# david8862/tf-keras-deeplabv3p-model-set

Hardware: AMD Instinct MI355X
Metric: images/sec (513x513, 21-class) MobileNetV2-DeepLabV3+ OS=16 training step (higher is better)
Workload: dtype f32

## Files before the change

tf-keras-deeplabv3p-model-set_amd/csrc/pw_gemm.h:

```cpp
#pragma once
#include "common.h"

struct GemmParams {
  const float* A; int lda;
  const float* scale; const float* shift; int act;
  const float* B; int ldb;
  const float* bias;
  float* Y; int ldy;
  float* partials;
  int M, K, N;
  int accumulate;
  int num_m_tiles;
  int ksplit, kchunk;
  int stagger;
  int b_kn;
  const float* bb_z; int bb_ldz;
  const float* bb_scale; const float* bb_shift; const float* bb_mean; const float* bb_invstd; int bb_act;
  int g_RH, g_RW, g_SH, g_SW, g_C, g_kw, g_mul, g_ay, g_ax, g_d, g_shift;
  uint32_t g_cmagic;
  int g_kwmagic;
  const unsigned short* Bsp; int bsp_pitch; long long bsp_plane;
  const float* f_z; int f_ldz; const float* f_scale; const float* f_shift; const float* f_mean; const float* f_invstd;
  const float* f_coef; int f_act; float* f_dz; int f_lddz;
};
```

tf-keras-deeplabv3p-model-set_amd/csrc/pw_split.hip:

```cpp
#include "common.h"
#include "pw_gemm.h"
#include "sb_common.h"

__global__ __launch_bounds__(256) void split_bf16x3_kernel(const float* src, unsigned short* dst, const long long* table) {
  const long long* e = table + (size_t)blockIdx.x * 6;
  const long long soff = e[0], doff = e[4];
  const int rows = (int)e[1], cols = (int)e[2], ld = (int)e[3], pitch = (int)e[5];
  const int p8 = pitch / 8;
  const long long plane = (long long)rows * pitch;
  for (long long i = (long long)blockIdx.y * 256 + threadIdx.x; i < (long long)rows * p8; i += (long long)gridDim.y * 256) {
    const int r = (int)(i / p8), c = (int)(i - (long long)r * p8) * 8;
    const long long so = soff + (long long)r * ld + c;
    float v[8];
    if (c + 8 <= cols && (so & 3) == 0) {
      const float4 a = *reinterpret_cast<const float4*>(src + so), b = *reinterpret_cast<const float4*>(src + so + 4);
      v[0] = a.x; v[1] = a.y; v[2] = a.z; v[3] = a.w; v[4] = b.x; v[5] = b.y; v[6] = b.z; v[7] = b.w;
    } else {
#pragma unroll
      for (int k = 0; k < 8; ++k) v[k] = c + k < cols ? src[so + k] : 0.f;
    }
    uint4 h, m, l;
    split2(v[0], v[1], h.x, m.x, l.x);
    split2(v[2], v[3], h.y, m.y, l.y);
    split2(v[4], v[5], h.z, m.z, l.z);
// ... 712 lines not shown
    default: if (mi == 1) launch_sbp_one<8, STATS, 1, BNB>(p, grid, st); else launch_sbp_one<8, STATS, 2, BNB>(p, grid, st); break;
  }
#undef DL3P_SBP
}

void dl3p_launch_gemm_sbp(const GemmParams& p, bool stats, bool bnb, int nt, int mi, dim3 grid, hipStream_t st) {
  if (bnb) launch_sbp_nt<true, true>(p, nt, mi, grid, st);
  else if (stats) launch_sbp_nt<true, false>(p, nt, mi, grid, st);
  else launch_sbp_nt<false, false>(p, nt, mi, grid, st);
}

template <int NT, bool STATS, int MI, bool BNB, bool GA, int WM>
static void launch_sb_one(const GemmParams& p, dim3 grid, hipStream_t st) {
  constexpr int BM = 64 * MI * WM, BN = 16 * NT;
  constexpr int OPER = 3 * (BM + BN) * SB_PB * 2;
  constexpr int TPP = NT < 4 ? NT : 4;
  constexpr int ES = 4 * WM * 16 * MI * (16 * TPP + 4) * 4;
  constexpr int RED = STATS ? 2 * 4 * WM * BN * 4 : 0;
  constexpr size_t lds = (size_t)(OPER > ES ? OPER : ES) + RED;
  static bool attr_set = false;
  if (!attr_set) {
    if (lds > 64 * 1024)
      (void)hipFuncSetAttribute((const void*)pw_gemm_sb_kernel<NT, STATS, MI, BNB, GA, WM>, hipFuncAttributeMaxDynamicSharedMemorySize, (int)lds);
    attr_set = true;
  }
  dl3p_launch(pw_gemm_sb_kernel<NT, STATS, MI, BNB, GA, WM>, grid, dim3(256 * WM), lds, st, p);
}

template <bool STATS, int MI, bool BNB, bool GA>
static void launch_sb_mi(const GemmParams& p, int nt, dim3 grid, hipStream_t st) {
  switch (nt) {
    case 1: launch_sb_one<1, STATS, MI, BNB, GA, 1>(p, grid, st); break;
    case 2: launch_sb_one<2, STATS, MI, BNB, GA, 1>(p, grid, st); break;
    case 3: launch_sb_one<3, STATS, MI, BNB, GA, 1>(p, grid, st); break;
    case 4: launch_sb_one<4, STATS, MI, BNB, GA, 1>(p, grid, st); break;
    case 5: launch_sb_one<5, STATS, MI, BNB, GA, 1>(p, grid, st); break;
    case 6: launch_sb_one<6, STATS, MI, BNB, GA, 1>(p, grid, st); break;
    case 7: launch_sb_one<7, STATS, MI, BNB, GA, 1>(p, grid, st); break;
    default: launch_sb_one<8, STATS, MI, BNB, GA, 1>(p, grid, st); break;
  }
}

template <bool STATS, bool BNB>
static void launch_sb_wide(const GemmParams& p, int nt, int mi, int wm, dim3 grid, hipStream_t st) {
#define DL3P_SBW(N_, M_, W_) if (nt == N_ && mi == M_ && wm == W_) { launch_sb_one<N_, STATS, M_, BNB, false, W_>(p, grid, st); return; }
  DL3P_SBW(16, 2, 1) DL3P_SBW(16, 1, 2) DL3P_SBW(16, 2, 2) DL3P_SBW(12, 2, 1) DL3P_SBW(12, 2, 2) DL3P_SBW(8, 2, 2) DL3P_SBW(16, 1, 1)
#undef DL3P_SBW
  launch_sb_one<16, STATS, 2, BNB, false, 1>(p, grid, st);
}

bool dl3p_sb_wide_config(int nt, int mi, int wm) {
  static const int ok[][3] = {{16, 2, 1}, {16, 1, 2}, {16, 2, 2}, {12, 2, 1}, {12, 2, 2}, {8, 2, 2}, {16, 1, 1}};
  for (auto& c : ok) if (c[0] == nt && c[1] == mi && c[2] == wm) return true;
  return false;
}

void dl3p_launch_gemm_sb(const GemmParams& p, bool stats, bool bnb, bool ga, int nt, int mi, int wm, dim3 grid, hipStream_t st) {
  if (wm > 1 || nt > 8) {
    if (bnb) launch_sb_wide<true, true>(p, nt, mi, wm, grid, st);
    else if (stats) launch_sb_wide<true, false>(p, nt, mi, wm, grid, st);
    else launch_sb_wide<false, false>(p, nt, mi, wm, grid, st);
    return;
  }
#define DL3P_SB(S, B, G) \
  { if (mi == 1) launch_sb_mi<S, 1, B, G>(p, nt, grid, st); else launch_sb_mi<S, 2, B, G>(p, nt, grid, st); return; }
  if (ga) {
    if (stats) DL3P_SB(true, false, true) else DL3P_SB(false, false, true)
  }
  if (bnb) DL3P_SB(true, true, false)
  if (stats) DL3P_SB(true, false, false)
  DL3P_SB(false, false, false)
#undef DL3P_SB
}

struct WgradSB {
  const float* X; int ldx; const float* scale; const float* shift; int act;
  const float* DY; int lddy;
  float* slabs;
  int M, K, N;
  int ktiles, ntiles, mrows;
  int k_base;
  int g_RH, g_RW, g_SH, g_SW, g_C, g_kw, g_mul, g_ay, g_ax, g_d;
  float g_invRW, g_invRH;
};

__device__ __forceinline__ int sb_divmod(int a, int d, float inv, int* r) {
  int q = (int)((float)a * inv);
  int rem = a - q * d;
  if (rem < 0) { --q; rem += d; }
  if (rem >= d) { ++q; rem -= d; }
  *r = rem;
  return q;
}

typedef short s16x4w __attribute__((ext_vector_type(4)));
__device__ __forceinline__ s16x4w tr_read16(const unsigned short* lds_ptr) {
  return __builtin_amdgcn_ds_read_tr16_b64_v4i16((s16x4w __attribute__((address_space(3)))*)lds_ptr);
}

template <int KF, int NW, int WN, bool GX = false>
__global__ __launch_bounds__(256, 2) void pw_wgrad_sb_kernel(WgradSB p) {
  constexpr int TK = 64 * KF, TN = 16 * NW, MS = 32;
  constexpr int KFW = KF * WN, NWW = NW / WN;
  constexpr int XP = TK + 8, DP = TN + 8;
  constexpr int X_PLANE = MS * XP, D_PLANE = MS * DP;
  constexpr int XCPR = TK / 8, DCPR = TN / 8;
  constexpr int XROWS = 256 / XCPR, DROWS = 256 / DCPR;
  constexpr int NXP = MS / XROWS, NDP = MS / DROWS;
  extern __shared__ __attribute__((aligned(16))) unsigned short wg_lds[];
  unsigned short* Xs = wg_lds;
  unsigned short* Ds = wg_lds + 3 * X_PLANE;
  const int t = threadIdx.x, l = t & 63, w = t >> 6;
  const int wk = w / WN, wn = w - wk * WN;
  const int tile = blockIdx.x, kt = tile / p.ntiles, nt = tile - kt * p.ntiles;
  const int k0 = p.k_base + kt * TK, n0 = nt * TN;
  const int mbeg = blockIdx.y * p.mrows, mend = min(p.M, mbeg + p.mrows);
  const int xm = t / XCPR, xc = (t - xm * XCPR) * 8;
  const int dm = t / DCPR, dc = (t - dm * DCPR) * 8;
  const int xk = k0 + xc, dn = n0 + dc;
  const bool xok0 = xk < p.K, xok1 = xk + 4 < p.K, dok0 = dn < p.N, dok1 = dn + 4 < p.N;
  const int xk0 = min(xk, p.K - 4), xk1 = min(xk + 4, p.K - 4), dn0 = min(dn, p.N - 4), dn1 = min(dn + 4, p.N - 4);
  const float* scp = p.scale ? p.scale : p.X;
  const float* shp = p.scale ? p.shift : p.X;
  int gc[2] = {xk0, xk1}, gdy[2] = {0, 0}, gdx[2] = {0, 0};
  if (GX) {
#pragma unroll
    for (int h = 0; h < 2; ++h) {
      const int k = h ? xk1 : xk0;
      const int tap = k / p.g_C, ky = tap / p.g_kw;
      gc[h] = k - tap * p.g_C;
      gdy[h] = p.g_ay + ky * p.g_d;
      gdx[h] = p.g_ax + (tap - ky * p.g_kw) * p.g_d;
    }
  }
  const float4 sc0 = ld4(scp + gc[0]), sc1 = ld4(scp + gc[1]), sh0 = ld4(shp + gc[0]), sh1 = ld4(shp + gc[1]);
  const float act_lo = p.act == DL3P_ACT_NONE ? -DL3P_INF : 0.f;
  const float act_hi = (p.act == DL3P_ACT_NONE || p.act == DL3P_ACT_RELU) ? DL3P_INF : 6.f;
  auto prologue4 = [&](float4 v, float4 sc4, float4 sh4) __attribute__((always_inline)) {
    if (p.scale) v = fma4(v, sc4, sh4);
    if (p.act >= DL3P_ACT_HSWISH) return act_apply4(v, p.act);
    return make_float4(__builtin_amdgcn_fmed3f(v.x, act_lo, act_hi), __builtin_amdgcn_fmed3f(v.y, act_lo, act_hi),
                       __builtin_amdgcn_fmed3f(v.z, act_lo, act_hi), __builtin_amdgcn_fmed3f(v.w, act_lo, act_hi));
  };
  const bool has_pro = p.scale != nullptr || p.act != DL3P_ACT_NONE;
  uint32_t gx_ok = 0;

  f32x4 acc[KFW][NWW];
#pragma unroll
  for (int kf = 0; kf < KFW; ++kf)
#pragma unroll
    for (int ni = 0; ni < NWW; ++ni) acc[kf][ni] = (f32x4){0.f, 0.f, 0.f, 0.f};
  float4 rx[NXP][2], rd[NDP][2];
  auto prefetch = [&](int m0) __attribute__((always_inline)) {
#pragma unroll
    for (int i = 0; i < NXP; ++i) {
      if (GX) {
        const int m = m0 + xm + XROWS * i;
        int x, y;
        const int row = sb_divmod(min(m, p.M - 1), p.g_RW, p.g_invRW, &x);
        const int n = sb_divmod(row, p.g_RH, p.g_invRH, &y);
        const uint32_t img = (uint32_t)n * (uint32_t)(p.g_SH * p.g_SW);
#pragma unroll
        for (int h = 0; h < 2; ++h) {
          const int sy = y * p.g_mul + gdy[h], sx = x * p.g_mul + gdx[h];
          const bool ok = m < mend && sy >= 0 && sx >= 0 && sy < p.g_SH && sx < p.g_SW;
          const uint32_t off = ok ? (img + (uint32_t)(sy * p.g_SW + sx)) * (uint32_t)p.ldx + (uint32_t)gc[h] : 0u;
          rx[i][h] = ld4(p.X + off);
          gx_ok = (gx_ok & ~(1u << (2 * i + h))) | (ok ? (1u << (2 * i + h)) : 0u);
        }
      } else {
        const float* xr = p.X + (size_t)min(m0 + xm + XROWS * i, p.M - 1) * p.ldx;
        rx[i][0] = ld4(xr + xk0); rx[i][1] = ld4(xr + xk1);
      }
    }
#pragma unroll
    for (int i = 0; i < NDP; ++i) {
      const float* dr = p.DY + (size_t)min(m0 + dm + DROWS * i, p.M - 1) * p.lddy;
      rd[i][0] = ld4(dr + dn0); rd[i][1] = ld4(dr + dn1);
    }
  };
  const int g = l >> 4, q = (l & 15) >> 2, pp = l & 3;
  const int r0 = (8 * g + q), r1 = (8 * g + 4 + q);
  const int nsteps = (mend - mbeg + MS - 1) / MS;
  if (nsteps > 0) prefetch(mbeg);
  for (int s = 0; s < nsteps; ++s) {
    const int m0 = mbeg + s * MS;
#pragma unroll
    for (int i = 0; i < NXP; ++i) {
      float4 v0 = rx[i][0], v1 = rx[i][1];
      if (has_pro) { v0 = prologue4(v0, sc0, sh0); v1 = prologue4(v1, sc1, sh1); }
      const bool rok = m0 + xm + XROWS * i < mend;
      const bool ok0 = GX ? ((gx_ok >> (2 * i)) & 1u) != 0 : rok, ok1 = GX ? ((gx_ok >> (2 * i + 1)) & 1u) != 0 : rok;
      if (!(ok0 && xok0)) v0 = zero4();
      if (!(ok1 && xok1)) v1 = zero4();
      uint4 hh, mm, ll;
      split2(v0.x, v0.y, hh.x, mm.x, ll.x);
      split2(v0.z, v0.w, hh.y, mm.y, ll.y);
      split2(v1.x, v1.y, hh.z, mm.z, ll.z);
      split2(v1.z, v1.w, hh.w, mm.w, ll.w);
      unsigned short* d = Xs + (xm + XROWS * i) * XP + xc;
      *reinterpret_cast<uint4*>(d) = hh;
      *reinterpret_cast<uint4*>(d + X_PLANE) = mm;
      *reinterpret_cast<uint4*>(d + 2 * X_PLANE) = ll;
    }
#pragma unroll
    for (int i = 0; i < NDP; ++i) {
      float4 v0 = rd[i][0], v1 = rd[i][1];
      const bool rok = m0 + dm + DROWS * i < mend;
      if (!(rok && dok0)) v0 = zero4();
      if (!(rok && dok1)) v1 = zero4();
      uint4 hh, mm, ll;
      split2(v0.x, v0.y, hh.x, mm.x, ll.x);
      split2(v0.z, v0.w, hh.y, mm.y, ll.y);
      split2(v1.x, v1.y, hh.z, mm.z, ll.z);
      split2(v1.z, v1.w, hh.w, mm.w, ll.w);
      unsigned short* d = Ds + (dm + DROWS * i) * DP + dc;
      *reinterpret_cast<uint4*>(d) = hh;
      *reinterpret_cast<uint4*>(d + D_PLANE) = mm;
      *reinterpret_cast<uint4*>(d + 2 * D_PLANE) = ll;
    }
    lds_barrier();
    prefetch(mbeg + min(s + 1, nsteps - 1) * MS);
    s16x8 af[KFW][3];
#pragma unroll
    for (int kf = 0; kf < KFW; ++kf)
#pragma unroll
      for (int pl = 0; pl < 3; ++pl) {
        const unsigned short* b = Xs + pl * X_PLANE + (wk * KFW + kf) * 16 + 4 * pp;
        const s16x4w a0 = tr_read16(b + r0 * XP), a1 = tr_read16(b + r1 * XP);
        af[kf][pl] = (s16x8){a0[0], a0[1], a0[2], a0[3], a1[0], a1[1], a1[2], a1[3]};
      }
#pragma unroll
    for (int ni = 0; ni < NWW; ++ni) {
      s16x8 bf[3];
#pragma unroll
      for (int pl = 0; pl < 3; ++pl) {
        const unsigned short* b = Ds + pl * D_PLANE + (wn * NWW + ni) * 16 + 4 * pp;
        const s16x4w b0 = tr_read16(b + r0 * DP), b1 = tr_read16(b + r1 * DP);
        bf[pl] = (s16x8){b0[0], b0[1], b0[2], b0[3], b1[0], b1[1], b1[2], b1[3]};
      }
#pragma unroll
      for (int kf = 0; kf < KFW; ++kf) {
        acc[kf][ni] = split_mac(acc[kf][ni], af[kf][0], af[kf][1], af[kf][2], bf[0], bf[1], bf[2]);
      }
    }
    lds_barrier();
  }
  float* slab = p.slabs + (size_t)blockIdx.y * p.K * p.N;
#pragma unroll
  for (int kf = 0; kf < KFW; ++kf)
#pragma unroll
    for (int ni = 0; ni < NWW; ++ni) {
      const int n = n0 + (wn * NWW + ni) * 16 + (l & 15);
#pragma unroll
      for (int j = 0; j < 4; ++j) {
        const int k = k0 + (wk * KFW + kf) * 16 + 4 * g + j;
        if (k < p.K && n < p.N) slab[(size_t)k * p.N + n] = acc[kf][ni][j];
      }
    }
}

int dl3p_wgrad_sb_plan(int M, int K, int N, int max_slabs, int tile, int per_cu, int* kf, int* nw, int* ktiles, int* ntiles, int* mrows) {
  if (M < 1024 || K < 32 || N < 32 || K % 4 || N % 4 || max_slabs < 1) return 0;
  static const int cand[5][2] = {{2, 8}, {1, 8}, {2, 4}, {1, 4}, {2, 16}};
  float best = 1e30f;
  for (int i = 0; i < (tile == 4 ? 5 : 4); ++i) {
    const int tk = 64 * cand[i][0], tn = 16 * cand[i][1];
    const float area = (float)((K + tk - 1) / tk * tk) * (float)((N + tn - 1) / tn * tn);
    const float cost = area * (1.f + 0.5f * (64.f / tk + 64.f / tn));
    if ((tile < 0 && cost < best) || tile == i) { best = cost; *kf = cand[i][0]; *nw = cand[i][1]; }
  }
  *ktiles = (K + 64 * *kf - 1) / (64 * *kf);
  *ntiles = (N + 16 * *nw - 1) / (16 * *nw);
  const int tiles = *ktiles * *ntiles;
  if (per_cu <= 0) per_cu = (*kf == 2 && *nw == 8) ? 2 : 4;
  int s = (DL3P_NUM_CUS * per_cu) / tiles;
  if (s < 1) s = 1;
  const int max_s = (M + 255) / 256;
  if (s > max_s) s = max_s;
  if (s > max_slabs) s = max_slabs;
  const int chunk = ((M + s - 1) / s + 31) / 32 * 32;
  *mrows = chunk;
  return (M + chunk - 1) / chunk;
}

template <int KF, int NW, int WN, bool GX>
static void launch_wgrad_tile(const WgradSB& p, dim3 grid, hipStream_t st) {
  constexpr size_t lds = (size_t)3 * 32 * ((64 * KF + 8) + (16 * NW + 8)) * sizeof(unsigned short);
  static bool attr_set = false;
  if (!attr_set) {
    if (lds > 64 * 1024)
      (void)hipFuncSetAttribute((const void*)pw_wgrad_sb_kernel<KF, NW, WN, GX>, hipFuncAttributeMaxDynamicSharedMemorySize, (int)lds);
    attr_set = true;
  }
  dl3p_launch(pw_wgrad_sb_kernel<KF, NW, WN, GX>, grid, dim3(256), lds, st, p);
}

void dl3p_launch_wgrad_sb(const float* x, int ldx, const float* scale, const float* shift, int act, const float* dy, int lddy,
                          float* slabs, int M, int K, int N, int kf, int nw, int ktiles, int ntiles, int mrows, int splits, hipStream_t st) {
  WgradSB p = {x, ldx, scale, shift, act, dy, lddy, slabs, M, K, N, ktiles, ntiles, mrows, 0};
  const dim3 block(256);
  if (kf == 2 && nw == 8) {
    const int rem = K % 128;
    static const int mixed = getenv("DL3P_WGRAD_SB_MIXED") ? atoi(getenv("DL3P_WGRAD_SB_MIXED")) : 0;
    if (mixed && rem > 0 && rem <= 64 && ktiles > 1) {
      p.ktiles = ktiles - 1;
      launch_wgrad_tile<2, 8, 2, false>(p, dim3(p.ktiles * ntiles, splits), st);
      p.k_base = 128 * (ktiles - 1);
      p.ktiles = 1;
      launch_wgrad_tile<1, 8, 1, false>(p, dim3(ntiles, splits), st);
      return;
    }
    launch_wgrad_tile<2, 8, 2, false>(p, dim3(ktiles * ntiles, splits), st);
  } else if (kf == 2 && nw == 16) launch_wgrad_tile<2, 16, 2, false>(p, dim3(ktiles * ntiles, splits), st);
  else if (kf == 1 && nw == 8) launch_wgrad_tile<1, 8, 1, false>(p, dim3(ktiles * ntiles, splits), st);
  else if (kf == 2 && nw == 4) launch_wgrad_tile<2, 4, 1, false>(p, dim3(ktiles * ntiles, splits), st);
  else launch_wgrad_tile<1, 4, 1, false>(p, dim3(ktiles * ntiles, splits), st);
}

void dl3p_launch_wgrad_sb_gx(const float* x, int ldx, const float* scale, const float* shift, int act, const float* dy, int lddy,
                             float* slabs, int M, int K, int N, const int* geo, int kf, int nw, int ktiles, int ntiles, int mrows, int splits,
                             hipStream_t st) {
  WgradSB p = {x, ldx, scale, shift, act, dy, lddy, slabs, M, K, N, ktiles, ntiles, mrows, 0};
  p.g_RH = geo[0]; p.g_RW = geo[1]; p.g_SH = geo[2]; p.g_SW = geo[3]; p.g_C = geo[4]; p.g_kw = geo[5]; p.g_mul = geo[6];
  p.g_ay = geo[7]; p.g_ax = geo[8]; p.g_d = geo[9];
  p.g_invRW = 1.f / (float)p.g_RW; p.g_invRH = 1.f / (float)p.g_RH;
  const dim3 grid(ktiles * ntiles, splits);
  if (kf == 2 && nw == 8) launch_wgrad_tile<2, 8, 2, true>(p, grid, st);
  else if (kf == 1 && nw == 8) launch_wgrad_tile<1, 8, 1, true>(p, grid, st);
  else if (kf == 2 && nw == 4) launch_wgrad_tile<2, 4, 1, true>(p, grid, st);
  else launch_wgrad_tile<1, 4, 1, true>(p, grid, st);
}
```

tf-keras-deeplabv3p-model-set_amd/csrc/pwconv.hip:

```cpp
#include "common.h"
#include <limits.h>
#include <type_traits>
#include <string.h>

typedef float f32x4 __attribute__((ext_vector_type(4)));

#define BK 32
#define APITCH 36

#include "pw_gemm.h"

#ifndef DL3P_GEMM_PIN_B
#define DL3P_GEMM_PIN_B 1
#endif
template <int NT, bool B_KN, bool STATS, int MI, int BKT, bool BNB = false, bool GA = false>
__global__ __launch_bounds__(256, 2) void pw_gemm_kernel(GemmParams p_in) {
  GemmParams p = p_in;
  int block_y = blockIdx.y;
#ifndef DL3P_NO_SPLITK
  if constexpr (!B_KN && !STATS && !BNB && !GA) {
    if (p.ksplit > 1) {
      const int nbn = (int)gridDim.y / p.ksplit;
      const int z = block_y / nbn;
      block_y -= z * nbn;
// ... 1704 lines not shown
  static const int off = getenv("DL3P_WGRAD_SMALL") ? atoi(getenv("DL3P_WGRAD_SMALL")) == 0 : 0;
  if (off) return false;
  const int kt = ceil_div(K, 16), ntn = ceil_div(N, 16);
  int best = -1, best_tiles = 1 << 30;
  for (int i = 0; i < (int)(sizeof(list) / sizeof(list[0])); ++i)
    if (list[i].kt >= kt && list[i].ntn >= ntn && list[i].kt * list[i].ntn < best_tiles) { best = i; best_tiles = list[i].kt * list[i].ntn; }
  if (best < 0 || best_tiles > 2 * kt * ntn) return false;
  *out = list[best];
  return true;
}

template <bool BNA = false>
static void launch_wgrad_small_any(const WgradParams& p, SmallShape sh, int grid, hipStream_t st) {
#define DL3P_WS(a, b) if (sh.kt == a && sh.ntn == b) { launch_wgrad_small<a, b, BNA>(p, grid, st); return; }
  DL3P_WS(1, 2) DL3P_WS(2, 1) DL3P_WS(2, 2) DL3P_WS(1, 6) DL3P_WS(2, 3) DL3P_WS(2, 4) DL3P_WS(4, 2) DL3P_WS(6, 2)
  DL3P_WS(2, 6) DL3P_WS(2, 9) DL3P_WS(9, 2) DL3P_WS(2, 12) DL3P_WS(12, 2) DL3P_WS(4, 4)
#undef DL3P_WS
}

static void wgrad_pick_tile(int M, int K, int N, int* kw, int* nw) {
  static const int cand[4][2] = {{1, 4}, {2, 4}, {1, 8}, {2, 8}};
  static const int env_force = getenv("DL3P_WGRAD_TILE") ? atoi(getenv("DL3P_WGRAD_TILE")) : -1;
  int force = env_force;
  if (const GemmTuned* e = gemm_tuned_lookup(4, M, K, N)) force = e->nt;
  if (g_wgrad_force_tile >= 0) force = g_wgrad_force_tile;
  if (force < 0 && M < 65536) { *kw = 1; *nw = 4; return; }
  float best = 1e30f;
  for (int i = 0; i < 4; ++i) {
    if (force >= 0 && i != force) continue;
    const int tk = 64 * cand[i][0], tn = 16 * cand[i][1];
    const float area = (float)(ceil_div(K, tk) * tk) * (float)(ceil_div(N, tn) * tn);
    const float cost = area * (1.f + 0.5f * (64.f / tk + 64.f / tn));
    if (cost < best) { best = cost; *kw = cand[i][0]; *nw = cand[i][1]; }
  }
}

static void wgrad_split(int M, int K, int N, int* ktiles, int* ntiles, int* splits, int* mchunk) {
  int kw, nw;
  wgrad_pick_tile(M, K, N, &kw, &nw);
  *ktiles = ceil_div(K, 64 * kw);
  *ntiles = ceil_div(N, 16 * nw);
  const int tiles = *ktiles * *ntiles;
  static const int env_per_cu = getenv("DL3P_WGRAD_PER_CU") ? atoi(getenv("DL3P_WGRAD_PER_CU")) : 4;
  int per_cu = env_per_cu;
  if (const GemmTuned* e = gemm_tuned_lookup(4, M, K, N)) per_cu = e->mi;
  if (g_wgrad_force_per_cu) per_cu = g_wgrad_force_per_cu;
  int s = (DL3P_NUM_CUS * per_cu) / tiles;
  if (s < 1) s = 1;
  int max_s = ceil_div(M, 256);
  if (s > max_s) s = max_s;
  if (s > DL3P_MAX_STAT_ROWS) s = DL3P_MAX_STAT_ROWS;
  int chunk = ceil_div(ceil_div(M, s), 32) * 32;
  *splits = ceil_div(M, chunk);
  *mchunk = chunk;
}

template <bool GX = false, bool BNA = false>
static void launch_wgrad_tiled(const WgradParams& p, int splits, hipStream_t st) {
  int kw, nw;
  wgrad_pick_tile(p.M, p.K, p.N, &kw, &nw);
  const dim3 grid(p.ktiles * p.ntiles, splits), block(256);
  if (kw == 1 && nw == 4) dl3p_launch(pw_wgrad_kernel<1, 4, GX, BNA>, grid, block, 0, st, p);
  else if (kw == 2 && nw == 4) dl3p_launch(pw_wgrad_kernel<2, 4, GX, BNA>, grid, block, 0, st, p);
  else if (kw == 1 && nw == 8) dl3p_launch(pw_wgrad_kernel<1, 8, GX, BNA>, grid, block, 0, st, p);
  else dl3p_launch(pw_wgrad_kernel<2, 8, GX, BNA>, grid, block, 0, st, p);
}

__global__ __launch_bounds__(256) void colsum_kernel(const float* dy, int lddy, long long M, int C, int c4s, int px,
                                                     int nbx, float* partials) {
  const int b = blockIdx.x;
  const int slab = b / nbx;
  const int bx = b - slab * nbx;
  const int pl = threadIdx.x / c4s;
  const int cl = threadIdx.x - pl * c4s;
  const bool active = pl < px;
  const int cbase4 = slab * c4s;
  const int c = (cbase4 + cl) * 4;
  float4 acc[1] = {zero4()};
  if (active)
    for (long long m = (long long)bx * px + pl; m < M; m += (long long)nbx * px) acc[0] = add4(acc[0], ld4(dy + (size_t)m * lddy + c));
  block_reduce_store<1>(acc, active, pl, cl, c4s, px, cbase4, C, partials + (size_t)bx * C);
}

extern "C" size_t dl3p_pwconv_bwd_weight_workspace(int M, int K, int N) {
  if (M <= 0 || K <= 0 || N <= 0) return 0;
  int kt, nt, s, mc;
  wgrad_split(M, K, N, &kt, &nt, &s, &mc);
  size_t a = (size_t)s * K * N;
  SmallShape sh;
  if (wgrad_small_pick(K, N, &sh)) a = (size_t)wgrad_small_grid(M, sh.kt, sh.ntn) * K * N;
  else {
    int kf, nw, kt2, nt2, mrows;
    const size_t s2 = (size_t)wgrad_sb_route(M, K, N, DL3P_MAX_STAT_ROWS, &kf, &nw, &kt2, &nt2, &mrows) * K * N;
    if (s2 > a) a = s2;
  }
  size_t b = (size_t)512 * N;
  return (a > b ? a : b) * sizeof(float);
}

static int pwconv_bwd_weight_impl(const float* x, int ldx, const float* in_scale, const float* in_shift,
                                  int in_act, const float* dy, int lddy, float* gw, float* gb, float* workspace,
                                  size_t workspace_bytes, int M, int K, int N, int* rows_out, void* stream) {
  int rc = check_mat("dl3p_pwconv_bwd_weight", x, ldx, K);
  if (rc) return rc;
  rc = check_mat("dl3p_pwconv_bwd_weight", dy, lddy, N);
  if (rc) return rc;
  DL3P_CHECK_ARG((gw || rows_out) && workspace && aligned16(workspace) && M > 0, "dl3p_pwconv_bwd_weight: bad arguments");
  DL3P_CHECK_ARG(!rows_out || (!gb && !dl3p_pw_tiny_applies(M)),
                 "dl3p_pwconv_bwd_weight_slabs: no bias gradient and more than %d rows (use dl3p_pwconv_bwd_weight)", 64);
  const size_t need = dl3p_pwconv_bwd_weight_workspace(M, K, N);
  if (workspace_bytes < need) {
    dl3p_set_error("dl3p_pwconv_bwd_weight: workspace %zu < %zu bytes", workspace_bytes, need);
    return DL3P_EWORKSPACE;
  }
  hipStream_t st = (hipStream_t)stream;
  if (dl3p_pw_tiny_applies(M)) {
    DL3P_CHECK_ARG(aligned16(gw) && (!gb || aligned16(gb)), "dl3p_pwconv_bwd_weight: gw/gb must be 16-byte aligned");
    dl3p_pw_tiny_wgrad(x, ldx, in_scale, in_shift, in_act, dy, lddy, gw, gb, M, K, N, st);
    DL3P_CHECK_LAUNCH("dl3p_pwconv_bwd_weight");
    return DL3P_OK;
  }
  WgradParams p = {};
  p.X = x; p.ldx = ldx; p.scale = in_scale; p.shift = in_shift; p.act = in_act;
  p.DY = dy; p.lddy = lddy; p.slabs = workspace; p.M = M; p.K = K; p.N = N;
  int splits;
  SmallShape sh;
  if (M >= 16 && wgrad_small_pick(K, N, &sh) && (unsigned long long)M * (unsigned long long)(ldx > lddy ? ldx : lddy) * 4ull < (1ull << 32)) {
    splits = wgrad_small_grid(M, sh.kt, sh.ntn);
    launch_wgrad_small_any(p, sh, splits, st);
  } else {
    int kf, nw, kt2, nt2, mrows, s2 = 0;
    s2 = wgrad_sb_route(M, K, N, workspace_bytes / ((size_t)K * N * 4), &kf, &nw, &kt2, &nt2, &mrows);
    if (s2 > 0) {
      splits = s2;
      dl3p_launch_wgrad_sb(x, ldx, in_scale, in_shift, in_act, dy, lddy, workspace, M, K, N, kf, nw, kt2, nt2, mrows, s2, st);
    } else {
      wgrad_split(M, K, N, &p.ktiles, &p.ntiles, &splits, &p.mchunk);
      launch_wgrad_tiled<false>(p, splits, st);
    }
  }
  DL3P_CHECK_LAUNCH("dl3p_pwconv_bwd_weight");
  if (rows_out) { *rows_out = splits; return DL3P_OK; }
  rc = dl3p_reduce_rows_impl(workspace, splits, (size_t)K * N, gw, 0, st);
  if (rc) return rc;
  if (gb) {
    int c4s, px, nslab;
    pick_lanes(N, &c4s, &px, &nslab);
    long long need_b = ceil_div_ll(M, px);
    int nbx = (int)(need_b < 512 ? need_b : 512);
    hipLaunchKernelGGL(colsum_kernel, dim3(nbx * nslab), dim3(256), 0, st, dy, lddy, (long long)M, N, c4s, px, nbx,
                       workspace);
    DL3P_CHECK_LAUNCH("dl3p_pwconv_bwd_weight(colsum)");
    rc = dl3p_reduce_rows_impl(workspace, nbx, (size_t)N, gb, 0, st);
  }
  return rc;
}

extern "C" int dl3p_pwconv_bwd_weight(const float* x, int ldx, const float* in_scale, const float* in_shift,
                                      int in_act, const float* dy, int lddy, float* gw, float* gb, float* workspace,
                                      size_t workspace_bytes, int M, int K, int N, void* stream) {
  return pwconv_bwd_weight_impl(x, ldx, in_scale, in_shift, in_act, dy, lddy, gw, gb, workspace, workspace_bytes, M, K, N,
                                nullptr, stream);
}

extern "C" int dl3p_pwconv_bwd_weight_slabs(const float* x, int ldx, const float* in_scale, const float* in_shift,
                                            int in_act, const float* dy, int lddy, float* workspace, size_t workspace_bytes,
                                            int* rows_out, int M, int K, int N, void* stream) {
  DL3P_CHECK_ARG(rows_out != nullptr, "dl3p_pwconv_bwd_weight_slabs: rows_out is required");
  return pwconv_bwd_weight_impl(x, ldx, in_scale, in_shift, in_act, dy, lddy, nullptr, nullptr, workspace, workspace_bytes, M, K,
                                N, rows_out, stream);
}


static int wgrad_bn_route(int M, int K, int N) {
  SmallShape sh;
  if (M <= 64 || dl3p_pw_tiny_applies(M) || N % 4 || K % 4) return 0;
  if (M >= 16 && wgrad_small_pick(K, N, &sh)) return (sh.kt == 2 && sh.ntn == 12) ? 0 : 1;
  int kw, nw;
  wgrad_pick_tile(M, K, N, &kw, &nw);
  return (K <= 64 * kw && !(kw == 2 && nw == 8)) ? 2 : 0;
}

extern "C" int dl3p_pwconv_bwd_weight_bn_supported(int M, int K, int N) { return wgrad_bn_route(M, K, N) != 0; }

extern "C" int dl3p_pwconv_bwd_weight_slabs_bn(const float* x, int ldx, const float* in_scale, const float* in_shift,
                                               int in_act, const float* g, int ldg, const float* z, int ldz,
                                               const float* bn_scale, const float* bn_shift, int bn_act,
                                               const float* save_mean, const float* save_invstd, const float* coef,
                                               float* dz, int lddz, float* workspace, size_t workspace_bytes,
                                               int* rows_out, int M, int K, int N, void* stream) {
  const char* fn = "dl3p_pwconv_bwd_weight_slabs_bn";
  int rc = check_mat(fn, x, ldx, K);
  if (rc) return rc;
  rc = check_mat(fn, g, ldg, N);
  if (rc) return rc;
  rc = check_mat(fn, z, ldz, N);
  if (rc) return rc;
  if (dz) {
    rc = check_mat(fn, dz, lddz, N);
    if (rc) return rc;
  }
  DL3P_CHECK_ARG(rows_out && workspace && aligned16(workspace) && save_mean && save_invstd && coef && dz != g,
                 "%s: bad arguments", fn);
  DL3P_CHECK_ARG(dl3p_pwconv_bwd_weight_bn_supported(M, K, N), "%s: shape M=%d K=%d N=%d is not served by the tiled kernel", fn,
                 M, K, N);
  const int ldmax = ldx > ldg ? (ldx > ldz ? ldx : ldz) : (ldg > ldz ? ldg : ldz);
  DL3P_CHECK_ARG((unsigned long long)M * (unsigned long long)(ldmax > lddz ? ldmax : lddz) * 4ull < (1ull << 32),
                 "%s: operands of 4 GiB or more are not supported (M=%d)", fn, M);
  const size_t need = dl3p_pwconv_bwd_weight_workspace(M, K, N);
  if (workspace_bytes < need) {
    dl3p_set_error("%s: workspace %zu < %zu bytes", fn, workspace_bytes, need);
    return DL3P_EWORKSPACE;
  }
  WgradParams p = {};
  p.X = x; p.ldx = ldx; p.scale = in_scale; p.shift = in_shift; p.act = in_act;
  p.DY = g; p.lddy = ldg; p.slabs = workspace; p.M = M; p.K = K; p.N = N;
  p.Z = z; p.ldz = ldz; p.b_scale = bn_scale; p.b_shift = bn_shift; p.b_mean = save_mean; p.b_invstd = save_invstd;
  p.b_coef = coef; p.b_act = bn_act; p.DZ = dz; p.lddz = lddz;
  int splits;
  SmallShape sh;
  if (wgrad_bn_route(M, K, N) == 1 && wgrad_small_pick(K, N, &sh)) {
    splits = wgrad_small_grid(M, sh.kt, sh.ntn);
    launch_wgrad_small_any<true>(p, sh, splits, (hipStream_t)stream);
  } else {
    wgrad_split(M, K, N, &p.ktiles, &p.ntiles, &splits, &p.mchunk);
    launch_wgrad_tiled<false, true>(p, splits, (hipStream_t)stream);
  }
  DL3P_CHECK_LAUNCH(fn);
  *rows_out = splits;
  return DL3P_OK;
}


static int conv_gemm_check(const char* fn, int N, int H, int W, int Cin, int Cout, int k, int stride, int rate, int pad_t,
                           int pad_l, int Ho, int Wo) {
  DL3P_CHECK_ARG(dl3p_conv2d_gemm_supported(Cin, Cout, k, stride), "%s: unsupported conv (Cin=%d Cout=%d k=%d stride=%d)", fn,
                 Cin, Cout, k, stride);
  DL3P_CHECK_ARG(N > 0 && H > 0 && W > 0 && Ho > 0 && Wo > 0 && rate > 0 && pad_t >= 0 && pad_l >= 0, "%s: bad geometry", fn);
  DL3P_CHECK_ARG((long long)N * H * W < (1ll << 24) && (long long)N * Ho * Wo < (1ll << 24) && H < 16384 && W < 16384,
                 "%s: tensor too large", fn);
  DL3P_CHECK_ARG((Ho - 1) * stride - pad_t < H && (Wo - 1) * stride - pad_l < W, "%s: output larger than the strided input", fn);
  return DL3P_OK;
}

extern "C" int dl3p_conv2d_gemm_supported(int Cin, int Cout, int k, int stride) {
  static const int enabled = getenv("DL3P_CONV_GEMM") ? atoi(getenv("DL3P_CONV_GEMM")) : 1;
  return enabled && Cin > 0 && Cout > 0 && Cin % 4 == 0 && Cout % 4 == 0 && k >= 1 && k <= 7 && (stride == 1 || stride == 2) &&
         (long long)k * k * Cin < 65536;
}

static void conv_gather_fwd(GemmParams* p, int H, int W, int Cin, int k, int stride, int rate, int pad_t, int pad_l, int Ho,
                            int Wo) {
  p->g_RH = Ho; p->g_RW = Wo; p->g_SH = H; p->g_SW = W; p->g_C = Cin; p->g_kw = k;
  p->g_mul = stride; p->g_ay = -pad_t; p->g_ax = -pad_l; p->g_d = rate; p->g_shift = 0;
  p->g_cmagic = (uint32_t)((1ull << 32) / (unsigned)Cin) + 1u;
  p->g_kwmagic = 65536 / k + 1;
}

extern "C" int dl3p_conv2d_gemm_fwd(const float* x, int ldx, const float* in_scale, const float* in_shift, int in_act,
                                    const float* wt, const float* bias, float* y, int ldy, float* stat_partials,
                                    int* rows_out, int N, int H, int W, int Cin, int Cout, int k, int stride, int rate,
                                    int pad_t, int pad_l, int Ho, int Wo, void* stream) {
  const char* fn = "dl3p_conv2d_gemm_fwd";
  int rc = conv_gemm_check(fn, N, H, W, Cin, Cout, k, stride, rate, pad_t, pad_l, Ho, Wo);
  if (rc) return rc;
  rc = check_mat(fn, x, ldx, Cin);
  if (rc) return rc;
  rc = check_mat(fn, y, ldy, Cout);
  if (rc) return rc;
  DL3P_CHECK_ARG(wt && aligned16(wt), "%s: bad kernel pointer", fn);
  const int M = N * Ho * Wo, K = k * k * Cin;
  DL3P_CHECK_ARG((unsigned long long)N * H * W * (unsigned long long)ldx * 4ull < (1ull << 32) &&
                     (unsigned long long)M * (unsigned long long)ldy * 4ull < (1ull << 32),
                 "%s: operands of 4 GiB or more are not supported", fn);
  GemmParams p = {};
  p.A = x; p.lda = ldx; p.scale = in_scale; p.shift = in_shift; p.act = in_act;
  p.B = wt; p.ldb = K; p.bias = bias; p.Y = y; p.ldy = ldy; p.partials = stat_partials;
  p.M = M; p.K = K; p.N = Cout;
  conv_gather_fwd(&p, H, W, Cin, k, stride, rate, pad_t, pad_l, Ho, Wo);
  const int nt = pick_nt(Cout, M);
  int gx, gy, mi;
  gemm_grid(M, Cout, nt, &gx, &gy, &p.num_m_tiles, &mi);
  if (rows_out) *rows_out = gx;
  if (stat_partials) launch_gemm<false, true, false, true>(p, nt, mi, dim3(gx, gy), (hipStream_t)stream);
  else launch_gemm<false, false, false, true>(p, nt, mi, dim3(gx, gy), (hipStream_t)stream);
  DL3P_CHECK_LAUNCH(fn);
  return DL3P_OK;
}

__global__ void conv_dgrad_weights_kernel(const float* w, float* wd, int taps, int Cin, int Cout) {
  const int total = taps * Cin * Cout;
  for (int i = blockIdx.x * 256 + threadIdx.x; i < total; i += gridDim.x * 256) {
    const int co = i % Cout, r = i / Cout;
    const int ci = r % Cin, tap = r / Cin;
    wd[((size_t)ci * taps + tap) * Cout + co] = w[i];
  }
}

extern "C" int dl3p_conv2d_gemm_dgrad_weights(const float* w, float* wd, int k, int Cin, int Cout, void* stream) {
  DL3P_CHECK_ARG(w && wd && k >= 1 && Cin > 0 && Cout > 0, "dl3p_conv2d_gemm_dgrad_weights: bad arguments");
  const int total = k * k * Cin * Cout;
  hipLaunchKernelGGL(conv_dgrad_weights_kernel, dim3(ceil_div(total, 256) < 1024 ? ceil_div(total, 256) : 1024), dim3(256), 0,
                     (hipStream_t)stream, w, wd, k * k, Cin, Cout);
  DL3P_CHECK_LAUNCH("dl3p_conv2d_gemm_dgrad_weights");
// ... 260 lines not shown
```

Before: 1364.

## Fuse BN-backward fold into split-bf16 wgrad kernel for mid-K pointwise convs

Adds a FOLD variant of the split-bf16 weight-gradient kernel that reads the pre-BN output z and applies the batch-norm/activation backward transform to dy on the fly, optionally writing dz from the k0==0 tile. A new route (3) sends BN-fused wgrad shapes with K in (64,192] that previously fell back to the generic tiled path into this kernel, with its own slab planning and workspace sizing. It also generalises the X-row mapping so tiles with K=192 (KF=3) work by idling extra threads. The aim is to use the faster MFMA-based kernel for more layers and avoid a separate BN-backward pass, at the cost of extra z loads per tile.

```diff
diff --git a/tf-keras-deeplabv3p-model-set_amd/csrc/pw_gemm.h b/tf-keras-deeplabv3p-model-set_amd/csrc/pw_gemm.h
--- a/tf-keras-deeplabv3p-model-set_amd/csrc/pw_gemm.h
+++ b/tf-keras-deeplabv3p-model-set_amd/csrc/pw_gemm.h
@@ -23,3 +23,5 @@
   const float* f_z; int f_ldz; const float* f_scale; const float* f_shift; const float* f_mean; const float* f_invstd;
   const float* f_coef; int f_act; float* f_dz; int f_lddz;
 };
+
+#define DL3P_WGRAD_SB_FOLD_MAX_K 192
diff --git a/tf-keras-deeplabv3p-model-set_amd/csrc/pw_split.hip b/tf-keras-deeplabv3p-model-set_amd/csrc/pw_split.hip
--- a/tf-keras-deeplabv3p-model-set_amd/csrc/pw_split.hip
+++ b/tf-keras-deeplabv3p-model-set_amd/csrc/pw_split.hip
@@ -818,6 +818,9 @@
   int k_base;
   int g_RH, g_RW, g_SH, g_SW, g_C, g_kw, g_mul, g_ay, g_ax, g_d;
   float g_invRW, g_invRH;
+  const float* f_z; int f_ldz;
+  const float* f_scale; const float* f_shift; const float* f_mean; const float* f_invstd; const float* f_coef; int f_act;
+  float* f_dz; int f_lddz;
 };
 
 __device__ __forceinline__ int sb_divmod(int a, int d, float inv, int* r) {
@@ -834,14 +837,15 @@
   return __builtin_amdgcn_ds_read_tr16_b64_v4i16((s16x4w __attribute__((address_space(3)))*)lds_ptr);
 }
 
-template <int KF, int NW, int WN, bool GX = false>
+template <int KF, int NW, int WN, bool GX = false, bool FOLD = false>
 __global__ __launch_bounds__(256, 2) void pw_wgrad_sb_kernel(WgradSB p) {
   constexpr int TK = 64 * KF, TN = 16 * NW, MS = 32;
   constexpr int KFW = KF * WN, NWW = NW / WN;
   constexpr int XP = TK + 8, DP = TN + 8;
   constexpr int X_PLANE = MS * XP, D_PLANE = MS * DP;
   constexpr int XCPR = TK / 8, DCPR = TN / 8;
-  constexpr int XROWS = 256 / XCPR, DROWS = 256 / DCPR;
+  constexpr int XROWS = 256 / XCPR >= 32 ? 32 : (256 / XCPR >= 16 ? 16 : 8), DROWS = 256 / DCPR;
+  constexpr bool XALL = XCPR * XROWS == 256;
   constexpr int NXP = MS / XROWS, NDP = MS / DROWS;
   extern __shared__ __attribute__((aligned(16))) unsigned short wg_lds[];
   unsigned short* Xs = wg_lds;
@@ -852,6 +856,7 @@
   const int k0 = p.k_base + kt * TK, n0 = nt * TN;
   const int mbeg = blockIdx.y * p.mrows, mend = min(p.M, mbeg + p.mrows);
   const int xm = t / XCPR, xc = (t - xm * XCPR) * 8;
+  const bool xact = XALL || t < XCPR * XROWS;
   const int dm = t / DCPR, dc = (t - dm * DCPR) * 8;
   const int xk = k0 + xc, dn = n0 + dc;
   const bool xok0 = xk < p.K, xok1 = xk + 4 < p.K, dok0 = dn < p.N, dok1 = dn + 4 < p.N;
@@ -870,6 +875,31 @@
     }
   }
   const float4 sc0 = ld4(scp + gc[0]), sc1 = ld4(scp + gc[1]), sh0 = ld4(shp + gc[0]), sh1 = ld4(shp + gc[1]);
+  float4 fA[2], fC[2], fD[2], fsc[2], fsh[2];
+  if (FOLD) {
+#pragma unroll
+    for (int h = 0; h < 2; ++h) {
+      const int cc = h ? dn1 : dn0;
+      const float4 one = make_float4(1.f, 1.f, 1.f, 1.f);
+      fsc[h] = p.f_scale ? ld4(p.f_scale + cc) : one;
+      fsh[h] = p.f_shift ? ld4(p.f_shift + cc) : zero4();
+      const float4 mu = ld4(p.f_mean + cc), is = ld4(p.f_invstd + cc);
+      const float4 c0 = ld4(p.f_coef + cc), c1 = ld4(p.f_coef + p.N + cc), c2 = ld4(p.f_coef + 2 * p.N + cc);
+      fA[h] = c0;
+      fC[h] = make_float4(c0.x * is.x * c2.x, c0.y * is.y * c2.y, c0.z * is.z * c2.z, c0.w * is.w * c2.w);
+      fD[h] = make_float4(fC[h].x * mu.x - c0.x * c1.x, fC[h].y * mu.y - c0.y * c1.y, fC[h].z * mu.z - c0.z * c1.z,
+                          fC[h].w * mu.w - c0.w * c1.w);
+    }
+  }
+  const bool write_dz = FOLD && p.f_dz != nullptr && k0 == 0;
+  auto fold4 = [&](float4 v, float4 z, int h) __attribute__((always_inline)) {
+    const float4 u = fma4(z, fsc[h], fsh[h]);
+    const int act = p.f_act;
+    return make_float4(fmaf(fA[h].x, v.x * act_grad(u.x, act), fmaf(-fC[h].x, z.x, fD[h].x)),
+                       fmaf(fA[h].y, v.y * act_grad(u.y, act), fmaf(-fC[h].y, z.y, fD[h].y)),
+                       fmaf(fA[h].z, v.z * act_grad(u.z, act), fmaf(-fC[h].z, z.z, fD[h].z)),
+                       fmaf(fA[h].w, v.w * act_grad(u.w, act), fmaf(-fC[h].w, z.w, fD[h].w)));
+  };
   const float act_lo = p.act == DL3P_ACT_NONE ? -DL3P_INF : 0.f;
   const float act_hi = (p.act == DL3P_ACT_NONE || p.act == DL3P_ACT_RELU) ? DL3P_INF : 6.f;
   auto prologue4 = [&](float4 v, float4 sc4, float4 sh4) __attribute__((always_inline)) {
@@ -886,10 +916,11 @@
   for (int kf = 0; kf < KFW; ++kf)
 #pragma unroll
     for (int ni = 0; ni < NWW; ++ni) acc[kf][ni] = (f32x4){0.f, 0.f, 0.f, 0.f};
-  float4 rx[NXP][2], rd[NDP][2];
+  float4 rx[NXP][2], rd[NDP][2], rz[FOLD ? NDP : 1][2];
   auto prefetch = [&](int m0) __attribute__((always_inline)) {
 #pragma unroll
     for (int i = 0; i < NXP; ++i) {
+      if (!xact) break;
       if (GX) {
         const int m = m0 + xm + XROWS * i;
         int x, y;
@@ -913,6 +944,10 @@
     for (int i = 0; i < NDP; ++i) {
       const float* dr = p.DY + (size_t)min(m0 + dm + DROWS * i, p.M - 1) * p.lddy;
       rd[i][0] = ld4(dr + dn0); rd[i][1] = ld4(dr + dn1);
+      if (FOLD) {
+        const float* zr = p.f_z + (size_t)min(m0 + dm + DROWS * i, p.M - 1) * p.f_ldz;
+        rz[i][0] = ld4(zr + dn0); rz[i][1] = ld4(zr + dn1);
+      }
     }
   };
   const int g = l >> 4, q = (l & 15) >> 2, pp = l & 3;
@@ -923,6 +958,7 @@
     const int m0 = mbeg + s * MS;
 #pragma unroll
     for (int i = 0; i < NXP; ++i) {
+      if (!xact) break;
       float4 v0 = rx[i][0], v1 = rx[i][1];
       if (has_pro) { v0 = prologue4(v0, sc0, sh0); v1 = prologue4(v1, sc1, sh1); }
       const bool rok = m0 + xm + XROWS * i < mend;
@@ -943,6 +979,14 @@
     for (int i = 0; i < NDP; ++i) {
       float4 v0 = rd[i][0], v1 = rd[i][1];
       const bool rok = m0 + dm + DROWS * i < mend;
+      if (FOLD) {
+        v0 = fold4(v0, rz[i][0], 0); v1 = fold4(v1, rz[i][1], 1);
+        if (write_dz && rok) {
+          float* dzr = p.f_dz + (size_t)(m0 + dm + DROWS * i) * p.f_lddz;
+          if (dok0) st4(dzr + dn, v0);
+          if (dok1) st4(dzr + dn + 4, v1);
+        }
+      }
       if (!(rok && dok0)) v0 = zero4();
       if (!(rok && dok1)) v1 = zero4();
       uint4 hh, mm, ll;
@@ -1020,16 +1064,16 @@
   return (M + chunk - 1) / chunk;
 }
 
-template <int KF, int NW, int WN, bool GX>
+template <int KF, int NW, int WN, bool GX, bool FOLD = false>
 static void launch_wgrad_tile(const WgradSB& p, dim3 grid, hipStream_t st) {
   constexpr size_t lds = (size_t)3 * 32 * ((64 * KF + 8) + (16 * NW + 8)) * sizeof(unsigned short);
   static bool attr_set = false;
   if (!attr_set) {
     if (lds > 64 * 1024)
-      (void)hipFuncSetAttribute((const void*)pw_wgrad_sb_kernel<KF, NW, WN, GX>, hipFuncAttributeMaxDynamicSharedMemorySize, (int)lds);
+      (void)hipFuncSetAttribute((const void*)pw_wgrad_sb_kernel<KF, NW, WN, GX, FOLD>, hipFuncAttributeMaxDynamicSharedMemorySize, (int)lds);
     attr_set = true;
   }
-  dl3p_launch(pw_wgrad_sb_kernel<KF, NW, WN, GX>, grid, dim3(256), lds, st, p);
+  dl3p_launch(pw_wgrad_sb_kernel<KF, NW, WN, GX, FOLD>, grid, dim3(256), lds, st, p);
 }
 
 void dl3p_launch_wgrad_sb(const float* x, int ldx, const float* scale, const float* shift, int act, const float* dy, int lddy,
@@ -1054,6 +1098,34 @@
   else launch_wgrad_tile<1, 4, 1, false>(p, dim3(ktiles * ntiles, splits), st);
 }
 
+int dl3p_wgrad_sb_fold_plan(int M, int K, int N, int max_slabs, int per_cu, int* ktiles, int* ntiles, int* mrows) {
+  if (M < 1024 || K <= 64 || K > DL3P_WGRAD_SB_FOLD_MAX_K || N < 32 || K % 4 || N % 4 || max_slabs < 1) return 0;
+  if (N <= 64 && M >= 16384) return 0;
+  if (M >= 65536) return 0;
+  *ktiles = 1;
+  *ntiles = (N + 63) / 64;
+  if (per_cu <= 0) per_cu = 2;
+  int s = (DL3P_NUM_CUS * per_cu) / *ntiles;
+  if (s < 1) s = 1;
+  const int max_s = (M + 255) / 256;
+  if (s > max_s) s = max_s;
+  if (s > max_slabs) s = max_slabs;
+  const int chunk = ((M + s - 1) / s + 31) / 32 * 32;
+  *mrows = chunk;
+  return (M + chunk - 1) / chunk;
+}
+
+void dl3p_launch_wgrad_sb_fold(const float* x, int ldx, const float* scale, const float* shift, int act, const float* g, int ldg,
+                               const float* z, int ldz, const float* bn_scale, const float* bn_shift, int bn_act, const float* mean,
+                               const float* invstd, const float* coef, float* dz, int lddz, float* slabs, int M, int K, int N,
+                               int ktiles, int ntiles, int mrows, int splits, hipStream_t st) {
+  WgradSB p = {x, ldx, scale, shift, act, g, ldg, slabs, M, K, N, ktiles, ntiles, mrows, 0};
+  p.f_z = z; p.f_ldz = ldz; p.f_scale = bn_scale; p.f_shift = bn_shift; p.f_mean = mean; p.f_invstd = invstd; p.f_coef = coef;
+  p.f_act = bn_act; p.f_dz = dz; p.f_lddz = lddz;
+  if (K <= 128) launch_wgrad_tile<2, 4, 1, false, true>(p, dim3(ktiles * ntiles, splits), st);
+  else launch_wgrad_tile<3, 4, 1, false, true>(p, dim3(ktiles * ntiles, splits), st);
+}
+
 void dl3p_launch_wgrad_sb_gx(const float* x, int ldx, const float* scale, const float* shift, int act, const float* dy, int lddy,
                              float* slabs, int M, int K, int N, const int* geo, int kf, int nw, int ktiles, int ntiles, int mrows, int splits,
                              hipStream_t st) {
diff --git a/tf-keras-deeplabv3p-model-set_amd/csrc/pwconv.hip b/tf-keras-deeplabv3p-model-set_amd/csrc/pwconv.hip
--- a/tf-keras-deeplabv3p-model-set_amd/csrc/pwconv.hip
+++ b/tf-keras-deeplabv3p-model-set_amd/csrc/pwconv.hip
@@ -1810,6 +1810,12 @@
   block_reduce_store<1>(acc, active, pl, cl, c4s, px, cbase4, C, partials + (size_t)bx * C);
 }
 
+int dl3p_wgrad_sb_fold_plan(int M, int K, int N, int max_slabs, int per_cu, int* ktiles, int* ntiles, int* mrows);
+static int wgrad_sb_fold_slabs(int M, int K, int N, size_t max_slabs, int* kt, int* nt, int* mrows) {
+  if (max_slabs > (size_t)DL3P_MAX_STAT_ROWS) max_slabs = DL3P_MAX_STAT_ROWS;
+  return dl3p_wgrad_sb_fold_plan(M, K, N, (int)max_slabs, g_sbw_force_pc, kt, nt, mrows);
+}
+
 extern "C" size_t dl3p_pwconv_bwd_weight_workspace(int M, int K, int N) {
   if (M <= 0 || K <= 0 || N <= 0) return 0;
   int kt, nt, s, mc;
@@ -1821,6 +1827,8 @@
     int kf, nw, kt2, nt2, mrows;
     const size_t s2 = (size_t)wgrad_sb_route(M, K, N, DL3P_MAX_STAT_ROWS, &kf, &nw, &kt2, &nt2, &mrows) * K * N;
     if (s2 > a) a = s2;
+    const size_t s3 = (size_t)wgrad_sb_fold_slabs(M, K, N, DL3P_MAX_STAT_ROWS, &kt2, &nt2, &mrows) * K * N;
+    if (s3 > a) a = s3;
   }
   size_t b = (size_t)512 * N;
   return (a > b ? a : b) * sizeof(float);
@@ -1900,13 +1908,24 @@
 }
 
 
+void dl3p_launch_wgrad_sb_fold(const float* x, int ldx, const float* scale, const float* shift, int act, const float* g, int ldg,
+                               const float* z, int ldz, const float* bn_scale, const float* bn_shift, int bn_act, const float* mean,
+                               const float* invstd, const float* coef, float* dz, int lddz, float* slabs, int M, int K, int N,
+                               int ktiles, int ntiles, int mrows, int splits, hipStream_t st);
+static int wgrad_sb_fold_route(int M, int K, int N, size_t max_slabs, int* kt, int* nt, int* mrows) {
+  const char* on = getenv("DL3P_FOLD_APPLY_SB");
+  if ((on && atoi(on) == 0) || !split_wgrad_on()) return 0;
+  return wgrad_sb_fold_slabs(M, K, N, max_slabs, kt, nt, mrows);
+}
 static int wgrad_bn_route(int M, int K, int N) {
   SmallShape sh;
   if (M <= 64 || dl3p_pw_tiny_applies(M) || N % 4 || K % 4) return 0;
   if (M >= 16 && wgrad_small_pick(K, N, &sh)) return (sh.kt == 2 && sh.ntn == 12) ? 0 : 1;
   int kw, nw;
   wgrad_pick_tile(M, K, N, &kw, &nw);
-  return (K <= 64 * kw && !(kw == 2 && nw == 8)) ? 2 : 0;
+  if (K <= 64 * kw && !(kw == 2 && nw == 8)) return 2;
+  int kt, nt, mrows;
+  return wgrad_sb_fold_route(M, K, N, DL3P_MAX_STAT_ROWS, &kt, &nt, &mrows) > 0 ? 3 : 0;
 }
 
 extern "C" int dl3p_pwconv_bwd_weight_bn_supported(int M, int K, int N) { return wgrad_bn_route(M, K, N) != 0; }
@@ -1930,6 +1949,7 @@
   }
   DL3P_CHECK_ARG(rows_out && workspace && aligned16(workspace) && save_mean && save_invstd && coef && dz != g,
                  "%s: bad arguments", fn);
+  const int route = wgrad_bn_route(M, K, N);
   DL3P_CHECK_ARG(dl3p_pwconv_bwd_weight_bn_supported(M, K, N), "%s: shape M=%d K=%d N=%d is not served by the tiled kernel", fn,
                  M, K, N);
   const int ldmax = ldx > ldg ? (ldx > ldz ? ldx : ldz) : (ldg > ldz ? ldg : ldz);
@@ -1947,7 +1967,13 @@
   p.b_coef = coef; p.b_act = bn_act; p.DZ = dz; p.lddz = lddz;
   int splits;
   SmallShape sh;
-  if (wgrad_bn_route(M, K, N) == 1 && wgrad_small_pick(K, N, &sh)) {
+  if (route == 3) {
+    int kt3, nt3, mrows;
+    splits = wgrad_sb_fold_route(M, K, N, workspace_bytes / ((size_t)K * N * 4), &kt3, &nt3, &mrows);
+    DL3P_CHECK_ARG(splits > 0, "%s: no plan for M=%d K=%d N=%d", fn, M, K, N);
+    dl3p_launch_wgrad_sb_fold(x, ldx, in_scale, in_shift, in_act, g, ldg, z, ldz, bn_scale, bn_shift, bn_act, save_mean, save_invstd,
+                              coef, dz, lddz, workspace, M, K, N, kt3, nt3, mrows, splits, (hipStream_t)stream);
+  } else if (route == 1 && wgrad_small_pick(K, N, &sh)) {
     splits = wgrad_small_grid(M, sh.kt, sh.ntn);
     launch_wgrad_small_any<true>(p, sh, splits, (hipStream_t)stream);
   } else {
```

After: 1374, median of 6. About the same (+0.7%).
